# imdea-software/legosnark

Measured on AMD Instinct MI355X. Metric: alt_bn128 G1 MSM point-scalar pairs/s at n=2^20, higher is better.
Workload: dtype u32 limbs (254-bit Montgomery integers)

## Files before the change

### legosnark_amd/csrc/msm.hip

```cpp
#include <hip/hip_runtime.h>
#include <stdint.h>
#include <stdio.h>
#include <stdlib.h>
#include <string.h>
#include <algorithm>
#include <type_traits>
#include <vector>

#include "curves.h"
#include "fp29x2l.h"
#include "fs29.h"
#include "glv.h"
#include "msm.h"
#include "msm_plan.h"

namespace lsa {


template <class F, int K>
__global__ __launch_bounds__(256) void k_normalize(const Jac<F> *__restrict__ in, Aff<F> *__restrict__ out, size_t n) {
    size_t t = (size_t)blockIdx.x * blockDim.x + threadIdx.x;
    size_t base = t * K;
    if (base >= n) return;
    F prod[K];
// ... 397 lines not shown
    const size_t lo = (size_t)t * tile;
    for (uint32_t il = threadIdx.x; il < tile; il += 1024) {
        const size_t i = lo + il;
        if (i >= n) break;
        const uint32_t seg = segment_of(segs, (uint32_t)i);
        const uint32_t local = (uint32_t)i - segs.off[seg];
        wide_digits(scalars[i], pl, seg * B, [&](unsigned k, int32_t sd) {
            if (sd != 0) {
                const uint32_t b = (uint32_t)(sd < 0 ? -sd : sd) - 1;
                const uint32_t ent = (local + k * win_stride) | (sd < 0 ? 0x80000000u : 0u);
                if (REC == 1) ((uint64_t *)out)[atomicAdd(&base[b >> 7], 1u)] = ((uint64_t)(b & 127u) << 32) | ent;
                else if (REC == 2) ((uint32_t *)out)[atomicAdd(&base[b >> 6], 1u)] = (ent & 0x81ffffffu) | ((b & 63u) << 25);
                else ((uint32_t *)out)[atomicAdd(&base[b], 1u)] = ent;
            }
        });
    }
}

__device__ __forceinline__ uint32_t lds_inc_rank(uint32_t *counters, uint32_t idx) {
    const uint32_t first = (uint32_t)__builtin_amdgcn_readfirstlane((int)idx);
    const uint64_t active = __ballot(1), same = __ballot(idx == first);
    if (same == active) {
        const uint32_t rank = __builtin_amdgcn_mbcnt_hi((uint32_t)(active >> 32), __builtin_amdgcn_mbcnt_lo((uint32_t)active, 0u));
        uint32_t base = 0;
        if (rank == 0) base = atomicAdd(&counters[first], (uint32_t)__popcll(active));
        return (uint32_t)__builtin_amdgcn_readfirstlane((int)base) + rank;
    }
    return atomicAdd(&counters[idx], 1u);
}
__global__ __launch_bounds__(1024) void k_partition(const Fr *__restrict__ scalars, size_t n, SegList segs, WidePlan pl, uint32_t B, uint32_t Bc,
                                                    CoarseMap cm, uint32_t pitch, const uint16_t *__restrict__ tile_hist,
                                                    const uint32_t *__restrict__ hist_c, uint32_t *__restrict__ offs_c,
                                                    const uint32_t *__restrict__ tile_base, uint32_t *__restrict__ recs) {
    __builtin_amdgcn_s_setprio(3);
    extern __shared__ __attribute__((aligned(16))) uint32_t stage[];
    __shared__ uint32_t lstart[PART_SEGS + 1], lcur[PART_SEGS], gdst[PART_SEGS], wtot[2][PART_SEGS / 64];
    const uint32_t t = xcd_tile(blockIdx.x, gridDim.x);
    const unsigned lane = threadIdx.x & 63, wv = threadIdx.x >> 6;
    {
        uint32_t gv = 0, lv = 0;
        if (threadIdx.x < Bc) { gv = hist_c[threadIdx.x]; lv = tile_hist[(size_t)t * pitch + threadIdx.x]; }
        uint32_t gi = gv, li = lv;
#pragma unroll
        for (int d = 1; d < 64; d <<= 1) {
            const uint32_t a = __shfl_up(gi, d, 64), b = __shfl_up(li, d, 64);
            if ((int)lane >= d) { gi += a; li += b; }
        }
        if (wv < PART_SEGS / 64 && lane == 63) { wtot[0][wv] = gi; wtot[1][wv] = li; }
        __syncthreads();
        if (threadIdx.x < Bc) {
            uint32_t gex = gi - gv, lex = li - lv;
            for (unsigned w = 0; w < wv; w++) { gex += wtot[0][w]; lex += wtot[1][w]; }
            lstart[threadIdx.x] = lex;
            lcur[threadIdx.x] = lex;
            gdst[threadIdx.x] = gex + tile_base[(size_t)t * pitch + threadIdx.x];
            if (blockIdx.x == 0) offs_c[threadIdx.x] = gex;
            if (threadIdx.x == Bc - 1) lstart[Bc] = lex + lv;
        }
    }
    __syncthreads();
    const size_t lo = (size_t)t * PART_TILE;
    const uint32_t fine_bits = cm.sh_hi;
    const uint32_t tlow = t & ((1u << (16 - fine_bits)) - 1);
    for (uint32_t j = 0; j < PART_TILE / 1024; j++) {
        const uint32_t il = threadIdx.x + j * 1024;
        const size_t i = lo + il;
        if (i >= n) break;
        const uint32_t seg = segment_of(segs, (uint32_t)i);
        wide_digits(scalars[i], pl, seg * B, [&](unsigned k, int32_t sd) {
            if (sd != 0) {
                const uint32_t b = (uint32_t)(sd < 0 ? -sd : sd) - 1;
                const uint32_t pos = atomicAdd(&lcur[cm.bin(b)], 1u);
                stage[pos] = (tlow << (16 + fine_bits)) | (cm.fine(b) << 16) | (k << 12) | (sd < 0 ? 0x800u : 0u) | il;
            }
        });
    }
    __syncthreads();
    for (uint32_t sg = threadIdx.x >> 5; sg < Bc; sg += 32) {
        const uint32_t a = lstart[sg], e = lstart[sg + 1], g = gdst[sg];
        for (uint32_t x = a + (lane & 31); x < e; x += 32) recs[g + (x - a)] = stage[x];
    }
}

__global__ __launch_bounds__(1024) void k_fine_sort_part(const uint32_t *__restrict__ recs, const uint32_t *__restrict__ offs_c,
                                                         const uint32_t *__restrict__ hist_c, const uint32_t *__restrict__ tile_base,
                                                         uint32_t pitch, uint32_t T, CoarseMap cm, SegList segs, uint32_t win_stride, uint32_t stage_cap,
                                                         uint32_t *__restrict__ entries, uint32_t *__restrict__ hist, uint32_t *__restrict__ offs) {
    __builtin_amdgcn_s_setprio(3);
    extern __shared__ __attribute__((aligned(16))) uint32_t sm[];
    __shared__ uint32_t wsum[16];
    const uint32_t sg = blockIdx.x, lo = offs_c[sg], ns = hist_c[sg];
    const uint32_t fine_bits = cm.sh_hi, FM = 1u << fine_bits, fmask = FM - 1, tbits = 16 - fine_bits;
    const uint32_t F = 1u << cm.bits(sg), bucket0 = cm.first(sg);
    uint32_t *cnt = sm, *cur = sm + FM, *col = sm + 2 * FM, *stage = col + T + 1;
    const unsigned lane = threadIdx.x & 63, wv = threadIdx.x >> 6;
    for (uint32_t x = threadIdx.x; x < F; x += 1024) cnt[x] = 0;
    for (uint32_t x = threadIdx.x; x < T; x += 1024) col[x] = tile_base[(size_t)x * pitch + sg];
    if (threadIdx.x == 0) col[T] = ns;
    auto scan_counters = [&]() {
        const uint32_t per = (F + 1023) >> 10, f0 = threadIdx.x * per;
        uint32_t sum = 0;
        for (uint32_t q = 0; q < per; q++) if (f0 + q < F) sum += cnt[f0 + q];
        uint32_t incl = sum;
#pragma unroll
        for (int d = 1; d < 64; d <<= 1) {
            const uint32_t u = __shfl_up(incl, d, 64);
            if ((int)lane >= d) incl += u;
        }
        if (lane == 63) wsum[wv] = incl;
        __syncthreads();
        uint32_t run = incl - sum;
        for (unsigned w = 0; w < wv; w++) run += wsum[w];
        for (uint32_t q = 0; q < per; q++) {
            if (f0 + q >= F) break;
            const uint32_t c = cnt[f0 + q];
            cur[f0 + q] = run;
            hist[(size_t)bucket0 + f0 + q] = c;
            offs[(size_t)bucket0 + f0 + q] = lo + run;
            run += c;
        }
    };
    auto entry_of = [&](uint32_t r, uint32_t p2) {
        uint32_t a = 0, e = (T + (1u << tbits) - 1) >> tbits;
        while (e - a > 1) {
            const uint32_t m = (a + e) >> 1;
            if (col[m << tbits] <= p2) a = m; else e = m;
        }
        const uint32_t i = ((a << tbits) | (r >> (16 + fine_bits))) * PART_TILE + (r & 0x7ffu);
        const uint32_t local = i - segs.off[segment_of(segs, i)];
        return (local + ((r >> 12) & 15u) * win_stride) | ((r & 0x800u) << 20);
    };
    if (ns <= stage_cap) {
        constexpr uint32_t NR = PART_STAGE / 1024;
        uint32_t r[NR];
#pragma unroll
        for (uint32_t u = 0; u < NR; u++) { const uint32_t p2 = threadIdx.x + u * 1024; r[u] = p2 < ns ? recs[lo + p2] : 0u; }
        __syncthreads();
        uint16_t rk[NR];
#pragma unroll
        for (uint32_t u = 0; u < NR; u++) {
            rk[u] = 0;
            if (threadIdx.x + u * 1024 < ns) rk[u] = (uint16_t)atomicAdd(&cnt[(r[u] >> 16) & fmask], 1u);
        }
        __syncthreads();
        scan_counters();
        __syncthreads();
#pragma unroll
        for (uint32_t u = 0; u < NR; u++) {
            const uint32_t p2 = threadIdx.x + u * 1024;
            if (p2 < ns) stage[cur[(r[u] >> 16) & fmask] + rk[u]] = entry_of(r[u], p2);
        }
        __syncthreads();
        for (uint32_t x = threadIdx.x; x < ns; x += 1024) entries[lo + x] = stage[x];
        return;
    }
    __syncthreads();
    constexpr uint32_t UNR = 8;
    for (uint32_t p0 = threadIdx.x; p0 < ns; p0 += 1024 * UNR) {
        uint32_t r[UNR];
#pragma unroll
        for (uint32_t u = 0; u < UNR; u++) { const uint32_t p2 = p0 + u * 1024; r[u] = p2 < ns ? recs[lo + p2] : 0u; }
#pragma unroll
        for (uint32_t u = 0; u < UNR; u++) if (p0 + u * 1024 < ns) (void)lds_inc_rank(cnt, (r[u] >> 16) & fmask);
    }
    __syncthreads();
    scan_counters();
    __syncthreads();
    for (uint32_t p0 = threadIdx.x; p0 < ns; p0 += 1024 * UNR) {
        uint32_t r[UNR];
#pragma unroll
        for (uint32_t u = 0; u < UNR; u++) { const uint32_t p2 = p0 + u * 1024; r[u] = p2 < ns ? recs[lo + p2] : 0u; }
#pragma unroll
        for (uint32_t u = 0; u < UNR; u++) {
            const uint32_t p2 = p0 + u * 1024;
            if (p2 >= ns) break;
            entries[lo + lds_inc_rank(cur, (r[u] >> 16) & fmask)] = entry_of(r[u], p2);
        }
    }
}

template <class Rec>
struct RecOps;
template <>
struct RecOps<uint64_t> {
    static constexpr uint32_t NF = 128;
    static __device__ __forceinline__ uint32_t fine(uint64_t r) { return (uint32_t)(r >> 32); }
    static __device__ __forceinline__ uint32_t entry(uint64_t r) { return (uint32_t)r; }
};
template <>
struct RecOps<uint32_t> {
    static constexpr uint32_t NF = 64;
    static __device__ __forceinline__ uint32_t fine(uint32_t r) { return (r >> 25) & 63u; }
    static __device__ __forceinline__ uint32_t entry(uint32_t r) { return r & 0x81ffffffu; }
};
template <class Rec>
__global__ __launch_bounds__(1024) void k_fine_sort(const Rec *__restrict__ recs, const uint32_t *__restrict__ offs_c,
                                                    const uint32_t *__restrict__ hist_c, uint32_t *__restrict__ entries,
                                                    uint32_t *__restrict__ hist, uint32_t *__restrict__ offs) {
    using O = RecOps<Rec>;
    constexpr uint32_t NF = O::NF;
    __shared__ uint32_t cnt[NF], cur[NF];
    const uint32_t bin = blockIdx.x, lo = offs_c[bin], n = hist_c[bin];
    if (threadIdx.x < NF) cnt[threadIdx.x] = 0;
    __syncthreads();
    for (uint32_t j = threadIdx.x; j < n; j += 1024) atomicAdd(&cnt[O::fine(recs[lo + j])], 1u);
    __syncthreads();
    if (threadIdx.x < 64) {
        constexpr uint32_t PER = NF / 64;
        uint32_t c[PER], tot = 0;
#pragma unroll
        for (uint32_t q = 0; q < PER; q++) { c[q] = cnt[PER * threadIdx.x + q]; tot += c[q]; }
        uint32_t incl = tot;
#pragma unroll
        for (int d = 1; d < 64; d <<= 1) {
            uint32_t t = __shfl_up(incl, d, 64);
            if ((int)threadIdx.x >= d) incl += t;
        }
        uint32_t ex = incl - tot;
#pragma unroll
        for (uint32_t q = 0; q < PER; q++) {
            cur[PER * threadIdx.x + q] = ex;
            hist[(size_t)bin * NF + PER * threadIdx.x + q] = c[q];
            offs[(size_t)bin * NF + PER * threadIdx.x + q] = lo + ex;
            ex += c[q];
        }
    }
    __syncthreads();
    for (uint32_t j = threadIdx.x; j < n; j += 1024) {
        const Rec r = recs[lo + j];
        const uint32_t pos = atomicAdd(&cur[O::fine(r)], 1u);
        entries[lo + pos] = O::entry(r);
    }
}

__device__ __forceinline__ uint32_t size_bin(uint32_t cnt, uint32_t bin_shift) { return ((cnt - 1) >> bin_shift) + 1; }
template <class C>
__global__ __launch_bounds__(256) void k_size_hist(const uint32_t *__restrict__ hist, uint32_t nb, uint32_t thr, uint32_t *__restrict__ bin_count,
                                                   uint32_t group_size, uint32_t bin_shift) {
    bin_count += (group_size ? (blockIdx.x * 2048u) / group_size : 0u) * SIZE_BINS;
    __shared__ uint32_t lcnt[SIZE_BINS];
    for (uint32_t t = threadIdx.x; t < SIZE_BINS; t += 256) lcnt[t] = 0;
    __syncthreads();
    const uint32_t base = blockIdx.x * 2048 + threadIdx.x;
#pragma unroll
    for (int j = 0; j < 8; j++) {
        uint32_t g = base + j * 256;
        if (g < nb) { uint32_t cnt = hist[g]; if (cnt > 0 && cnt <= thr) atomicAdd(&lcnt[size_bin(cnt, bin_shift)], 1u); }
    }
    __syncthreads();
    for (uint32_t t = threadIdx.x; t < SIZE_BINS; t += 256) if (lcnt[t]) atomicAdd(&bin_count[t], lcnt[t]);
}
__global__ __launch_bounds__(256) void k_size_scan(const uint32_t *__restrict__ bin_count, uint32_t *__restrict__ bin_start, uint32_t ngroups) {
    __shared__ uint32_t lds[4];
    uint32_t carry = 0;
    for (uint32_t gidx = 0; gidx < ngroups; gidx++) {
        const uint32_t *bc = bin_count + gidx * SIZE_BINS;
        uint32_t *bs = bin_start + gidx * SIZE_BINS;
        uint32_t v[4], s = 0;
#pragma unroll
        for (int j = 0; j < 4; j++) {
            int bin = (int)SIZE_BINS - 1 - (int)(threadIdx.x * 4 + j);
            v[j] = (bin >= 1) ? bc[bin] : 0;
            s += v[j];
        }
        uint32_t tot;
        uint32_t run = carry + block_exclusive_scan_256(s, lds, &tot);
#pragma unroll
        for (int j = 0; j < 4; j++) {
            int bin = (int)SIZE_BINS - 1 - (int)(threadIdx.x * 4 + j);
            if (bin >= 1) bs[bin] = run;
            run += v[j];
        }
        carry += tot;
    }
    if (threadIdx.x == 0) bin_start[0] = carry;
}
template <class C>
__global__ __launch_bounds__(256) void k_size_scatter(const uint32_t *__restrict__ hist, uint32_t nb, uint32_t thr, const uint32_t *__restrict__ bin_start,
                                                      uint32_t *__restrict__ bin_cursor, uint32_t *__restrict__ perm,
                                                      uint32_t *__restrict__ heavy_list, uint32_t *__restrict__ heavy_count,
                                                      typename C::Acc *__restrict__ buckets, uint32_t group_size, uint32_t bin_shift,
                                                      uint32_t split) {
    const uint32_t goff = (group_size ? (blockIdx.x * 2048u) / group_size : 0u) * SIZE_BINS;
    bin_start += goff;
    bin_cursor += goff;
    __shared__ uint32_t lcnt[SIZE_BINS];
    for (uint32_t t = threadIdx.x; t < SIZE_BINS; t += 256) lcnt[t] = 0;
    __syncthreads();
    const uint32_t base = blockIdx.x * 2048 + threadIdx.x;
    uint32_t cnt[8], rank[8];
#pragma unroll
    for (int j = 0; j < 8; j++) {
        uint32_t g = base + j * 256;
        cnt[j] = 0; rank[j] = 0;
        if (g < nb) {
            cnt[j] = hist[g];
            if (cnt[j] == 0) { for (uint32_t h = 0; h < split; h++) buckets[(size_t)g * split + h] = C::inf(); }
            else if (cnt[j] > thr) heavy_list[atomicAdd(heavy_count, 1u)] = g;
            else rank[j] = atomicAdd(&lcnt[size_bin(cnt[j], bin_shift)], 1u);
        }
    }
    __syncthreads();
    for (uint32_t t = threadIdx.x; t < SIZE_BINS; t += 256) {
        uint32_t c = lcnt[t];
        lcnt[t] = c ? atomicAdd(&bin_cursor[t], c) : 0;
    }
    __syncthreads();
#pragma unroll
    for (int j = 0; j < 8; j++) {
        uint32_t g = base + j * 256;
        if (g < nb && cnt[j] > 0 && cnt[j] <= thr) {
            const uint32_t bin = size_bin(cnt[j], bin_shift);
            perm[bin_start[bin] + lcnt[bin] + rank[j]] = g;
        }
    }
}

typedef uint32_t u32x4 __attribute__((ext_vector_type(4)));
template <class B> struct RawBase {
    static_assert(sizeof(B) % 16 == 0, "packed bases are whole 16-byte vectors");
    u32x4 q[sizeof(B) / 16];
};
template <class B>
__device__ __forceinline__ RawBase<B> load_base16(const B *__restrict__ p) {
    const u32x4 *src = reinterpret_cast<const u32x4 *>(p);
    RawBase<B> r;
#pragma unroll
    for (int i = 0; i < (int)(sizeof(B) / 16); i++) r.q[i] = src[i];
    return r;
}
template <class B>
__device__ __forceinline__ B packed_base(RawBase<B> r) {
    B b;
    uint32_t *dst = reinterpret_cast<uint32_t *>(&b);
#pragma unroll
    for (int i = 0; i < (int)(sizeof(B) / 16); i++) {
        asm("" : "+v"(r.q[i]));
        dst[4 * i] = r.q[i].x; dst[4 * i + 1] = r.q[i].y; dst[4 * i + 2] = r.q[i].z; dst[4 * i + 3] = r.q[i].w;
    }
    return b;
}
template <class C> struct RotatedLoads { static constexpr bool value = true; };
template <> struct RotatedLoads<CurveG2> { static constexpr bool value = false; };
template <class C, uint32_t ACC_SPLIT, bool ROTATED = RotatedLoads<C>::value>
__device__ __forceinline__ void accumulate_body(const typename C::Base *__restrict__ bases, const uint32_t *__restrict__ entries,
                                                const uint32_t *__restrict__ offs, const uint32_t *__restrict__ hist,
                                                const uint32_t *__restrict__ perm, const uint32_t *__restrict__ nperm,
                                                typename C::Acc *__restrict__ buckets) {
    uint32_t t = blockIdx.x * blockDim.x + threadIdx.x;
    if (t >= *nperm * ACC_SPLIT) return;
    const uint32_t g = perm[t / ACC_SPLIT], part = t % ACC_SPLIT;
    const uint32_t cnt = hist[g];
    const uint32_t *e = entries + offs[g];
    constexpr bool ENDO = ACC_SPLIT != 1;
    typename C::Acc acc = C::inf();
    if constexpr (!ROTATED) {
        if (part < cnt) {
            uint32_t v = e[part];
            typename C::Base cur = bases[v & 0x3fffffffu];
            static_assert(!C::HEAD || ROTATED, "the affine + affine head is written for the rotated loop only");
            for (uint32_t j = part; j < cnt; j += ACC_SPLIT) {
                uint32_t vn = v;
                typename C::Base nxt = cur;
                if (j + ACC_SPLIT < cnt) { vn = e[j + ACC_SPLIT]; nxt = bases[vn & 0x3fffffffu]; }
                acc = C::template madd<ENDO>(acc, cur, (v >> 31) != 0, ((v >> 30) & 1) != 0);
                v = vn;
                cur = nxt;
            }
        }
    } else if (part < cnt) {
        const uint32_t last = part + (cnt - 1 - part) / ACC_SPLIT * ACC_SPLIT;
        auto word = [&](uint32_t k) { return e[k < last ? k : last]; };
        auto base = [&](uint32_t w) { return load_base16(bases + (w & 0x3fffffffu)); };
        uint32_t j = part;
        uint32_t v = word(j), vn = word(j + ACC_SPLIT);
        RawBase<typename C::Base> cur;
        if constexpr (C::HEAD) {
            const uint32_t v2 = word(j + 2 * ACC_SPLIT), v3 = word(j + 3 * ACC_SPLIT);
            const RawBase<typename C::Base> r0 = base(v), r1 = base(vn), r2 = base(v2);
            const typename C::Base b0 = packed_base(r0), b1 = packed_base(r1);
            cur = r0;
            if (j + ACC_SPLIT < cnt && C::head_ok(b0, b1)) {
                acc = C::template madd_head<ENDO>(b0, (v >> 31) != 0, ((v >> 30) & 1) != 0, b1, (vn >> 31) != 0, ((vn >> 30) & 1) != 0);
                j += 2 * ACC_SPLIT;
                v = v2;
                vn = v3;
                cur = r2;
            }
        } else {
            cur = base(v);
        }
        for (; j < cnt; j += ACC_SPLIT) {
            const uint32_t vnn = word(j + 2 * ACC_SPLIT);
            const RawBase<typename C::Base> nxt = base(vn);
            acc = C::template madd<ENDO>(acc, packed_base(cur), (v >> 31) != 0, ((v >> 30) & 1) != 0);
            v = vn;
            vn = vnn;
            cur = nxt;
        }
    }
    buckets[(size_t)g * ACC_SPLIT + part] = acc;
}
template <class C, uint32_t ACC_SPLIT>
__global__ __launch_bounds__(256) void k_accumulate(const typename C::Base *__restrict__ bases, const uint32_t *__restrict__ entries,
                                                    const uint32_t *__restrict__ offs, const uint32_t *__restrict__ hist,
                                                    const uint32_t *__restrict__ perm, const uint32_t *__restrict__ nperm,
                                                    typename C::Acc *__restrict__ buckets) {
    accumulate_body<C, ACC_SPLIT>(bases, entries, offs, hist, perm, nperm, buckets);
}
__global__ __launch_bounds__(256) __attribute__((amdgpu_waves_per_eu(2, 2))) void k_accumulate_g2_occ2(
    const CurveG2::Base *__restrict__ bases, const uint32_t *__restrict__ entries, const uint32_t *__restrict__ offs,
    const uint32_t *__restrict__ hist, const uint32_t *__restrict__ perm, const uint32_t *__restrict__ nperm, CurveG2::Acc *__restrict__ buckets) {
    accumulate_body<CurveG2, 1u>(bases, entries, offs, hist, perm, nperm, buckets);
}

__global__ __launch_bounds__(256) void k_accumulate_g2_pair(const AffPackedG2 *__restrict__ bases, const uint32_t *__restrict__ entries,
                                                            const uint32_t *__restrict__ offs, const uint32_t *__restrict__ hist,
                                                            const uint32_t *__restrict__ perm, const uint32_t *__restrict__ nperm,
                                                            XYZZ29x2 *__restrict__ buckets) {
    const uint32_t t = blockIdx.x * blockDim.x + threadIdx.x, pr = t >> 1, part = t & 1;
    if (pr >= *nperm) return;
    const uint32_t g = perm[pr];
    const uint32_t cnt = hist[g];
    const uint32_t *e = entries + offs[g];
    struct Half { uint32_t x[8], y[8]; };
    auto fetch = [&](uint32_t v) {
        const AffPackedG2 &b = bases[v & 0x3fffffffu];
        Half h;
#pragma unroll
        for (int i = 0; i < 8; i++) { h.x[i] = b.w[part][i]; h.y[i] = b.w[2 + part][i]; }
        return h;
    };
    XyzzE<F29h> acc = XyzzE<F29h>::inf();
    uint32_t v = e[0];
    Half cur = fetch(v);
    for (uint32_t j = 0; j < cnt; j++) {
        uint32_t vn = v;
        Half nxt = cur;
        if (j + 1 < cnt) { vn = e[j + 1]; nxt = fetch(vn); }
        AffE<F29h> q = {{F29::unpack256(cur.x)}, {F29::unpack256(cur.y)}};
        if (!q.is_inf()) {
            if (v >> 31) q.y = sub_k<1>(F29h::zero(), q.y);
            acc = g2_madd(acc, q);
        }
        v = vn;
        cur = nxt;
    }
    F29 *o = reinterpret_cast<F29 *>(&buckets[g]);
    o[part] = acc.X.v;
    o[2 + part] = acc.Y.v;
    o[4 + part] = acc.ZZ.v;
    o[6 + part] = acc.ZZZ.v;
}

template <class A>
__device__ __forceinline__ A shfl_down_acc(const A &p, unsigned delta) {
    A r;
    constexpr int NW = sizeof(A) / 4;
    const uint32_t *src = reinterpret_cast<const uint32_t *>(&p);
    uint32_t *dst = reinterpret_cast<uint32_t *>(&r);
#pragma unroll
    for (int i = 0; i < NW; i++) dst[i] = __shfl_down(src[i], delta, 64);
    return r;
}

enum TailKernel { TAIL_HEAVY, TAIL_REDUCE1_LANE, TAIL_REDUCE2_LANE };
template <class C, TailKernel K> struct PairedAdd { static constexpr bool value = false; };
template <> struct PairedAdd<CurveG1, TAIL_HEAVY> { static constexpr bool value = true; };
template <> struct PairedAdd<CurveG1, TAIL_REDUCE1_LANE> { static constexpr bool value = true; };

template <class C, bool PAIRED = false>
__device__ __forceinline__ typename C::Acc wave_sum(typename C::Acc v, unsigned lane) {
    for (unsigned d = 32; d >= 1; d >>= 1) {
        typename C::Acc t = shfl_down_acc(v, d);
        if (lane + d < 64) v = C::template add<PAIRED>(v, t);
    }
    return v;
}

__global__ __launch_bounds__(256) void k_heavy_plan(const uint32_t *__restrict__ hist, const uint32_t *__restrict__ heavy_list,
                                                    const uint32_t *__restrict__ heavy_count, uint32_t *__restrict__ chunk_off) {
    __shared__ uint32_t lds[4];
    __shared__ uint32_t s_chunk;
    const uint32_t nh = *heavy_count;
    uint32_t carry = 0;
    for (uint32_t base = 0; base < nh; base += 256) {
        uint32_t h = base + threadIdx.x;
        uint32_t tot;
        (void)block_exclusive_scan_256(h < nh ? hist[heavy_list[h]] : 0, lds, &tot);
        carry += tot;
    }
    if (threadIdx.x == 0) {
        uint32_t chunk = HEAVY_CHUNK;
        while (chunk < 4096u && carry / (2 * chunk) >= 2048u) chunk *= 2;
        s_chunk = chunk;
    }
    __syncthreads();
    const uint32_t chunk = s_chunk;
    carry = 0;
    for (uint32_t base = 0; base < nh; base += 256) {
        uint32_t h = base + threadIdx.x;
        uint32_t v = h < nh ? (hist[heavy_list[h]] + chunk - 1) / chunk : 0;
        uint32_t tot;
        uint32_t ex = block_exclusive_scan_256(v, lds, &tot);
        if (h < nh) chunk_off[h] = carry + ex;
        carry += tot;
    }
    if (threadIdx.x == 0) { chunk_off[nh] = carry; chunk_off[nh + 1] = chunk; }
}

template <class C>
__global__ __launch_bounds__(64) void k_accumulate_heavy(const typename C::Base *__restrict__ bases, const uint32_t *__restrict__ entries,
                                                         const uint32_t *__restrict__ offs, const uint32_t *__restrict__ hist,
                                                         const uint32_t *__restrict__ heavy_list, const uint32_t *__restrict__ heavy_count,
                                                         const uint32_t *__restrict__ chunk_off, typename C::Acc *__restrict__ partials) {
    const uint32_t nh = *heavy_count;
    if (nh == 0) return;
    const uint32_t total = chunk_off[nh], chunk = chunk_off[nh + 1];
    const unsigned lane = threadIdx.x;
    for (uint32_t v = blockIdx.x; v < total; v += gridDim.x) {
        uint32_t lo = 0, hi = nh;
        while (hi - lo > 1) { uint32_t mid = (lo + hi) >> 1; if (chunk_off[mid] <= v) lo = mid; else hi = mid; }
        const uint32_t g = heavy_list[lo];
        const uint32_t cnt = hist[g];
        const uint32_t start = (v - chunk_off[lo]) * chunk;
        const uint32_t end = start + chunk < cnt ? start + chunk : cnt;
        const uint32_t *e = entries + offs[g];
        typename C::Acc acc = C::inf();
        uint32_t j = start + lane;
        if constexpr (!RotatedLoads<C>::value) {
            for (; j < end; j += 64) {
                uint32_t w = e[j];
                acc = C::madd(acc, bases[w & 0x3fffffffu], (w >> 31) != 0, ((w >> 30) & 1) != 0);
            }
        } else if (j < end) {
            const uint32_t last = j + (end - 1 - j) / 64 * 64;
            auto word = [&](uint32_t k) { return e[k < last ? k : last]; };
            uint32_t w = word(j), wn = word(j + 64);
            RawBase<typename C::Base> cur = load_base16(bases + (w & 0x3fffffffu));
            for (; j < end; j += 64) {
                const uint32_t wnn = word(j + 128);
                const RawBase<typename C::Base> nxt = load_base16(bases + (wn & 0x3fffffffu));
                acc = C::madd(acc, packed_base(cur), (w >> 31) != 0, ((w >> 30) & 1) != 0);
                w = wn;
                wn = wnn;
                cur = nxt;
            }
        }
        acc = wave_sum<C, PairedAdd<C, TAIL_HEAVY>::value>(acc, lane);
        if (lane == 0) partials[v] = acc;
    }
}

template <class C>
__global__ __launch_bounds__(64) void k_heavy_finish(const uint32_t *__restrict__ heavy_list, const uint32_t *__restrict__ heavy_count,
                                                     const uint32_t *__restrict__ chunk_off, const typename C::Acc *__restrict__ partials,
                                                     typename C::Acc *__restrict__ buckets, uint32_t split) {
    const uint32_t nh = *heavy_count;
    unsigned lane = threadIdx.x;
    for (uint32_t h = blockIdx.x; h < nh; h += gridDim.x) {
        typename C::Acc acc = C::inf();
        for (uint32_t v = chunk_off[h] + lane; v < chunk_off[h + 1]; v += 64) acc = C::add(acc, partials[v]);
        acc = wave_sum<C>(acc, lane);
        if (lane == 0) {
            buckets[(size_t)heavy_list[h] * split] = acc;
            for (uint32_t x = 1; x < split; x++) buckets[(size_t)heavy_list[h] * split + x] = C::inf();
        }
    }
}

template <class A>
__device__ __forceinline__ A select_acc(uint32_t mask, const A &a, const A &b) {
    A r;
    const uint32_t *pa = reinterpret_cast<const uint32_t *>(&a), *pb = reinterpret_cast<const uint32_t *>(&b);
    uint32_t *pr = reinterpret_cast<uint32_t *>(&r);
#pragma unroll
    for (int i = 0; i < (int)(sizeof(A) / 4); i++) pr[i] = (pa[i] & mask) | (pb[i] & ~mask);
    return r;
}
template <class A>
__device__ __forceinline__ void quadwave_weighted(A &acc, A &run, unsigned log_mult, unsigned lane) {
    const unsigned q = lane & 3, qi = lane >> 2;
    A s = A::inf();
#pragma unroll 1
    for (unsigned step = 0; step < 9; step++) {
        if (step == 4) {
            s = (qi == 0) ? A::inf() : run;
#pragma unroll 1
            for (unsigned i = 0; i < log_mult; i++) s = quad_dbl(s, q);
        }
        uint32_t m_run = step < 4 ? 0xffffffffu : 0u, m_s = step == 4 ? 0xffffffffu : 0u;
// ... 570 lines not shown
    (void)hipFree(tmp);
    if (rc) return rc;
    if (e != hipSuccess) { set_error("precompute_windows: %s", hipGetErrorString(e)); return LSA_ERR_HIP; }
    return LSA_OK;
}
template <class F>
int precompute_window_step(void *d_table, size_t n, void *d_tmp, unsigned k, hipStream_t st) {
    using C = typename CurveOf<F>::type;
    const TableGrid grid = table_grid(n);
    if (n == 0 || k == 0 || k >= grid.ncopies) return LSA_OK;
    typename C::Base *tbl = (typename C::Base *)d_table;
    hipLaunchKernelGGL((k_shift_window<C>), dim3((unsigned)((n + 255) / 256)), dim3(256), 0, st, tbl + (size_t)(k - 1) * n, (Jac<F> *)d_tmp, n, grid.pos[k] - grid.pos[k - 1]);
    return prepare_bases<F>((const Jac<F> *)d_tmp, tbl + (size_t)k * n, n, st);
}
template int precompute_window_step<Fq>(void *, size_t, void *, unsigned, hipStream_t);
template int precompute_window_step<Fq2>(void *, size_t, void *, unsigned, hipStream_t);
template int precompute_windows<Fq>(void *, size_t, hipStream_t);
template int precompute_windows<Fq2>(void *, size_t, hipStream_t);

unsigned msm_field_mults_per_pair(size_t n, size_t table_n) {
    if (table_n && n >= switches().table_use_min) return wide_plan(table_n, n, 1, switches()).nwin * 10;
    return 16 * 10 + 8;
}

template <class A>
struct MsmBuffers {
    uint32_t *hist, *heavy_count, *offs, *bsum, *bin_count, *bin_start, *bin_cursor, *perm;
    int32_t *digits;
    uint16_t *rank, *tile_hist;
    uint32_t *tile_base, *entries, *heavy_list, *chunk_off;
    A *hpart;
    void *recs;
    uint32_t *hist_c, *offs_c;
    A *buckets, *wave_out, *window_sums;
    void *res;

    MsmBuffers(const PipelinePlan &p, void *front_ws, void *tail_ws) {
        char *ws = (char *)front_ws, *tws = (char *)tail_ws;
        hist = (uint32_t *)(ws + p.front[F_HIST]);
        heavy_count = hist + p.nb;
        offs = (uint32_t *)(ws + p.front[F_OFFS]);
        bsum = (uint32_t *)(ws + p.front[F_BSUM]);
        bin_count = (uint32_t *)(ws + p.front[F_BINS]);
        bin_start = bin_count + SIZE_BINS;
        bin_cursor = bin_start + SIZE_BINS;
        perm = (uint32_t *)(ws + p.front[F_PERM]);
        digits = (int32_t *)(ws + p.front[F_DIGITS]);
        rank = (uint16_t *)(ws + p.front[F_RANK]);
        tile_hist = (uint16_t *)(ws + p.front[F_THIST]);
        tile_base = (uint32_t *)(ws + p.front[F_TBASE]);
        entries = (uint32_t *)(ws + p.front[F_ENTRIES]);
        heavy_list = (uint32_t *)(ws + p.front[F_HEAVY]);
        chunk_off = (uint32_t *)(ws + p.front[F_CHOFF]);
        hpart = (A *)(ws + p.front[F_HPART]);
        recs = ws + p.front[F_RECS];
        hist_c = p.fine ? (uint32_t *)(ws + p.front[F_CHIST]) : hist;
        offs_c = p.fine ? (uint32_t *)(ws + p.front[F_COFFS]) : offs;
        buckets = (A *)(tws + p.tail[T_BUCKETS]);
        wave_out = (A *)(tws + p.tail[T_WAVE]);
        window_sums = (A *)(tws + p.tail[T_WIN]);
        res = tws + p.tail[T_RES];
    }
};

struct Marks {
    hipEvent_t *ev;
    void operator()(int i, hipStream_t s) const { if (ev) (void)hipEventRecord(ev[i], s); }
};

template <class C>
static void launch_sort(const PipelinePlan &p, const MsmBuffers<typename C::Acc> &b, const Fr *d_scalars, const SegList &segs, hipStream_t st,
                        const Marks &mark) {
    const size_t n = p.n;
    if (p.wide) {
        hipLaunchKernelGGL(k_hist_wide, dim3(p.wtiles), dim3(1024), p.lds_hist_wide, st, d_scalars, n, segs, p.pl, p.B, p.Bc, p.cm, p.pitch, p.wtile, b.tile_hist);
        mark(1, st);
        hipLaunchKernelGGL(k_tile_scan_rows, dim3((p.Bc + 31) / 32), dim3(1024), 0, st, b.tile_hist, p.Bc, p.wtiles, p.pitch, b.tile_base, b.hist_c, b.heavy_count,
                           b.bin_count, (uint32_t)(3 * SIZE_BINS));
        mark(2, st);
        if (p.part) {
            hipLaunchKernelGGL(k_partition, dim3(p.wtiles), dim3(1024), p.lds_partition, st, d_scalars, n, segs, p.pl, p.B, p.Bc, p.cm, p.pitch,
                               b.tile_hist, b.hist_c, b.offs_c, b.tile_base, (uint32_t *)b.recs);
            hipLaunchKernelGGL(k_fine_sort_part, dim3(p.Bc), dim3(1024), p.lds_fine_sort_part, st, (const uint32_t *)b.recs, b.offs_c, b.hist_c,
                               b.tile_base, p.pitch, p.wtiles, p.cm, segs, p.win_stride, p.stage_cap, b.entries, b.hist, b.offs);
        } else if (p.rec32) {
            hipLaunchKernelGGL(k_scatter_wide<2>, dim3(p.wtiles), dim3(1024), p.lds_scatter_wide, st, d_scalars, n, segs, p.pl, p.B, p.Bc, p.pitch, p.wtile, b.hist_c, b.offs_c, b.tile_base, b.recs, p.win_stride);
            hipLaunchKernelGGL(k_fine_sort<uint32_t>, dim3(p.Bc), dim3(1024), 0, st, (const uint32_t *)b.recs, b.offs_c, b.hist_c, b.entries, b.hist, b.offs);
        } else if (p.fine) {
            hipLaunchKernelGGL(k_scatter_wide<1>, dim3(p.wtiles), dim3(1024), p.lds_scatter_wide, st, d_scalars, n, segs, p.pl, p.B, p.Bc, p.pitch, p.wtile, b.hist_c, b.offs_c, b.tile_base, b.recs, p.win_stride);
            hipLaunchKernelGGL(k_fine_sort<uint64_t>, dim3(p.Bc), dim3(1024), 0, st, (const uint64_t *)b.recs, b.offs_c, b.hist_c, b.entries, b.hist, b.offs);
        } else {
            hipLaunchKernelGGL(k_scatter_wide<0>, dim3(p.wtiles), dim3(1024), p.lds_scatter_wide, st, d_scalars, n, segs, p.pl, p.B, p.Bc, p.pitch, p.wtile, b.hist_c, b.offs_c, b.tile_base, (void *)b.entries, p.win_stride);
        }
        mark(3, st);
    } else {
        hipLaunchKernelGGL((k_digits<C::GLV>), dim3((unsigned)((n + 255) / 256)), dim3(256), 0, st, d_scalars, n, p.c, p.nwin, b.digits);
        hipLaunchKernelGGL(k_rank, dim3(p.ntiles, p.nwin), dim3(1024), p.lds_rank, st, b.digits, p.nv, p.B, p.ntiles, b.rank, b.tile_hist, 0u);
        hipLaunchKernelGGL(k_tile_scan, dim3((p.nb + 255) / 256), dim3(256), 0, st, b.tile_hist, p.B, p.ntiles, p.nb, b.tile_base, b.hist);
        mark(1, st);
        hipLaunchKernelGGL(k_scan_sums, dim3(p.scan_blocks), dim3(256), 0, st, b.hist, p.nb, b.bsum);
        hipLaunchKernelGGL(k_scan_blocks, dim3(1), dim3(256), 0, st, b.bsum, p.scan_blocks);
        hipLaunchKernelGGL(k_scan_final, dim3(p.scan_blocks), dim3(256), 0, st, b.hist, b.bsum, p.nb, b.offs);
        mark(2, st);
        hipLaunchKernelGGL(k_scatter, dim3(p.ntiles, p.nwin), dim3(1024), p.lds_scatter, st, b.digits, b.rank, b.offs, b.tile_base, p.nv, n, p.B, p.ntiles, b.entries, 0u);
        mark(3, st);
    }
}

template <class C>
static int launch_accumulate(const PipelinePlan &p, const MsmBuffers<typename C::Acc> &b, const typename C::Base *d_bases, hipStream_t st, const Marks &mark) {
    constexpr bool g2 = std::is_same<C, CurveG2>::value;
    if (!p.wide || p.reuse_sort) {
        HIPCHK(hipMemsetAsync(b.heavy_count, 0, 4, st));
        HIPCHK(hipMemsetAsync(b.bin_count, 0, (size_t)3 * SIZE_BINS * 4, st));
    }
    const unsigned sb = (p.nb + 2047) / 2048;
    const uint32_t gsz = 0u, ngroups = 1;
    hipLaunchKernelGGL((k_size_hist<C>), dim3(sb), dim3(256), 0, st, b.hist, p.nb, p.heavy_threshold, b.bin_count, gsz, p.bin_shift);
    hipLaunchKernelGGL(k_size_scan, dim3(1), dim3(256), 0, st, b.bin_count, b.bin_start, ngroups);
    hipLaunchKernelGGL((k_size_scatter<C>), dim3(sb), dim3(256), 0, st, b.hist, p.nb, p.heavy_threshold, b.bin_start, b.bin_cursor, b.perm, b.heavy_list, b.heavy_count, b.buckets, gsz, p.bin_shift, p.split);
    mark(4, st);
    const dim3 one_lane((p.nb + 255) / 256), two_lanes((p.nb * 2 + 255) / 256);
    if (g2 && p.g2_pair) {
        if constexpr (g2) hipLaunchKernelGGL(k_accumulate_g2_pair, two_lanes, dim3(256), 0, st, d_bases, b.entries, b.offs, b.hist, b.perm, b.bin_start, b.buckets);
    } else if (g2 && p.split == 1) {
        if constexpr (g2) hipLaunchKernelGGL(k_accumulate_g2_occ2, one_lane, dim3(256), 0, st, d_bases, b.entries, b.offs, b.hist, b.perm, b.bin_start, b.buckets);
    } else if (p.split == 1) {
        hipLaunchKernelGGL((k_accumulate<C, 1u>), one_lane, dim3(256), 0, st, d_bases, b.entries, b.offs, b.hist, b.perm, b.bin_start, b.buckets);
    } else {
        hipLaunchKernelGGL((k_accumulate<C, 2u>), two_lanes, dim3(256), 0, st, d_bases, b.entries, b.offs, b.hist, b.perm, b.bin_start, b.buckets);
    }
    hipLaunchKernelGGL(k_heavy_plan, dim3(1), dim3(256), 0, st, b.hist, b.heavy_list, b.heavy_count, b.chunk_off);
    hipLaunchKernelGGL((k_accumulate_heavy<C>), dim3(4096), dim3(64), 0, st, d_bases, b.entries, b.offs, b.hist,
                       b.heavy_list, b.heavy_count, b.chunk_off, b.hpart);
    hipLaunchKernelGGL((k_heavy_finish<C>), dim3(256), dim3(64), 0, st, b.heavy_list, b.heavy_count, b.chunk_off, b.hpart, b.buckets, p.split);
    mark(5, st);
    return LSA_OK;
}

template <class C>
static int launch_tail(const PipelinePlan &p, const MsmBuffers<typename C::Acc> &b, Jac<typename C::Field> *d_out, hipStream_t tail, bool inline_tail,
                       bool lane_l1, TailBuf &tb, TailBuf &prev, const Marks &mark) {
    using A = typename C::Acc;
    using J = Jac<typename C::Field>;
    constexpr bool g1 = std::is_same<C, CurveG1>::value;
    if (p.big)
        hipLaunchKernelGGL((k_reduce1_lane<C>), dim3(p.kw * ((p.T + 63) / 64)), dim3(64), 0, tail, b.buckets, p.B, p.L, p.split, b.wave_out);
    else
        hipLaunchKernelGGL((k_reduce1<C>), dim3(p.kw * p.wpw), dim3(64), 0, tail, b.buckets, p.B, p.L, p.logL, p.wpw, p.split, b.wave_out);
    A *lvl_in = b.wave_out, *lvl_out = b.window_sums;
    uint32_t m = p.wpw, lm = p.big ? p.logL : p.logL + 4;
    J *res = inline_tail ? d_out : (J *)b.res;
    const auto level = [&](bool lane) {
        const uint32_t m_out = (m + 15) / 16;
        if (lane) hipLaunchKernelGGL((k_reduce2_lane<C>), dim3((m_out + 63) / 64), dim3(64), 0, tail, lvl_in, m, m_out, lm, lvl_out);
        else hipLaunchKernelGGL((k_reduce2<C>), dim3(p.kw * m_out), dim3(64), 0, tail, lvl_in, m, m_out, lm, lvl_out);
        std::swap(lvl_in, lvl_out);
        m = m_out;
        lm += 4;
    };
    level(lane_l1);
    if (p.bits_tail) {
        uint32_t nbits = 0;
        while ((1u << nbits) < m) nbits++;
        const uint32_t G = (m + 511) / 512;
        A *part = lvl_out;
        A *weighted = part + (size_t)(nbits + 1) * G;
        hipLaunchKernelGGL((k_reduce_bits_a<C>), dim3(nbits + 1, G), dim3(512), 0, tail, lvl_in, m, nbits, G, part);
        hipLaunchKernelGGL((k_reduce_bits_b<C>), dim3(nbits + 1), dim3(64), 0, tail, part, nbits, G, lm, weighted);
        mark(6, tail);
        hipLaunchKernelGGL((k_reduce_bits_c<C>), dim3(1), dim3(64), 0, tail, weighted, nbits + 1, res);
    } else {
        while (m > 1) level(false);
        mark(6, tail);
        if (p.wide && p.nseg > 1) {
            if constexpr (g1) hipLaunchKernelGGL(k_emit_g1, dim3(p.nseg), dim3(64), 0, tail, lvl_in, res);
            else hipLaunchKernelGGL(k_emit_g2, dim3(p.nseg), dim3(64), 0, tail, lvl_in, res);
        } else if constexpr (g1) {
            hipLaunchKernelGGL(k_fold_quad, dim3(1), dim3(64), 0, tail, lvl_in, p.kw, p.c, res);
        } else {
            hipLaunchKernelGGL(k_fold_quad_g2, dim3(1), dim3(64), 0, tail, lvl_in, p.kw, p.c, res);
        }
    }
    if (!inline_tail) {
        int rc = publish_order_large(tb, prev, tail);
        if (rc) return rc;
        hipLaunchKernelGGL(k_publish, dim3(1), dim3(256), 0, tail, (const uint32_t *)res, (uint32_t *)d_out, (unsigned)(p.nseg * sizeof(J) / 4));
    }
    mark(7, tail);
    return LSA_OK;
}

static int plan_error(const PipelinePlan &p) {
    switch (p.status) {
    case PLAN_OK: return LSA_OK;
    case PLAN_N_TOO_LARGE: set_error("msm: n too large (%zu)", p.n); break;
    case PLAN_SEGMENTS_NEED_COPIES: set_error("msm: segmented calls need bases with pre-shifted copies"); break;
    case PLAN_TABLE_TOO_LARGE: set_error("msm: base table too large for 30-bit entries"); break;
    case PLAN_BIN_SPACE: set_error("msm: %u segments of %u buckets exceed the bin space", p.nseg, p.B); break;
    }
    return LSA_ERR_INVALID;
}

template <class F>
static int msm_pipeline(const void *d_bases_v, size_t first, const Fr *d_scalars, const SegList &segs, Jac<F> *d_out, hipStream_t st,
                        size_t table_stride, bool reuse_sort = false, bool blocking = false) {
    using C = typename CurveOf<F>::type;
    using A = typename C::Acc;
    const typename C::Base *d_bases = (const typename C::Base *)d_bases_v + first;
    const MsmShape shape = {std::is_same<C, CurveG1>::value ? 1 : 2, sizeof(A), sizeof(Jac<F>), C::GLV, segs.off[segs.nseg], segs.nseg,
                            table_stride, blocking, reuse_sort};
    const PipelinePlan p = plan_pipeline(shape, switches());
    int rc = plan_error(p);
    if (rc) return rc;
    if (g_ws.ensure(p.front.total) != 0) { set_error("msm: workspace allocation of %zu bytes failed", p.front.total); return LSA_ERR_NOMEM; }
// ... 101 lines not shown
```

### legosnark_amd/csrc/msm_plan.h

```cpp
#pragma once
#include <stdint.h>
#include <stddef.h>
#include "bn254_constants.h"
#include "fp.h"

namespace lsa {

struct WidePlan {
    unsigned nwin;
    unsigned c;
    unsigned copy_step;
    unsigned start[32];
    unsigned width[32];
};

struct TableGrid {
    unsigned ncopies;
    unsigned pos[33];
};
inline TableGrid table_grid(size_t n_table) {
    TableGrid t;
    const unsigned nbig = n_table >= ((size_t)6 << 20) ? 12u : 13u;
    const unsigned base = 255 / nbig, rem = 255 % nbig;
    unsigned bit = 0;
    for (unsigned k = 0; k < nbig; k++) {
        const unsigned w = base + (k < rem ? 1u : 0u);
        t.pos[2 * k] = bit;
        t.pos[2 * k + 1] = bit + (w + 1) / 2;
        bit += w;
    }
    t.ncopies = 2 * nbig;
    t.pos[t.ncopies] = 255;
    return t;
}

inline WidePlan wide_plan_for(size_t n_table, bool big) {
    const TableGrid t = table_grid(n_table);
    WidePlan pl = {};
    pl.copy_step = big ? 2 : 1;
    pl.nwin = t.ncopies / pl.copy_step;
    pl.c = 0;
    for (unsigned k = 0; k < pl.nwin; k++) {
        pl.start[k] = t.pos[k * pl.copy_step];
        pl.width[k] = t.pos[(k + 1) * pl.copy_step] - pl.start[k];
        if (pl.width[k] > pl.c) pl.c = pl.width[k];
    }
    return pl;
}

#define SORT_TILE 32768u
#define SCAN_PER_BLOCK 2048
#define WIDE_FINE_BITS 7u
#define MSM_MAX_SEGMENTS 64u
#define PART_TILE 2048u
#define PART_SEGS 768u
#define PART_STAGE 28672u
#define SIZE_BINS 1025
#define HEAVY_CHUNK 512u

constexpr uint32_t LDS_MAX_BIN_WORDS = 131072;
constexpr uint32_t LDS_MAX_BIN_HALVES = 65536;
constexpr uint32_t LDS_MAX_PARTITION = 13 * PART_TILE * 4;
constexpr uint32_t LDS_MAX_FINE_SORT_PART = 155648;

struct SegList {
    uint32_t nseg;
    uint32_t off[MSM_MAX_SEGMENTS + 1];
};

struct CoarseMap {
    uint32_t half, sh_lo, sh_hi, nlo;
    LSA_HD uint32_t bin(uint32_t b) const { return b < half ? b >> sh_lo : nlo + ((b - half) >> sh_hi); }
    LSA_HD uint32_t fine(uint32_t b) const { return b < half ? b & ((1u << sh_lo) - 1) : (b - half) & ((1u << sh_hi) - 1); }
    LSA_HD uint32_t first(uint32_t bin_) const { return bin_ < nlo ? bin_ << sh_lo : half + ((bin_ - nlo) << sh_hi); }
    LSA_HD uint32_t bits(uint32_t bin_) const { return bin_ < nlo ? sh_lo : sh_hi; }
};

inline unsigned msm_window_bits(size_t n) {
    unsigned lg = 0;
    while ((size_t(1) << (lg + 1)) <= n) lg++;
    int c = (int)lg - 4;
    if (c < 8) c = 8;
    if (c > 16) c = 16;
    return (unsigned)c;
}

inline unsigned num_windows(unsigned c) { return (255 + c - 1) / c; }

inline uint32_t wide_tile(uint32_t nwin, size_t n) {
    if (n <= 4096) return 256u;
    if (n <= 16384) return 1024u;
    return nwin > 15 ? 2048u : 4096u;
}

struct MsmSwitches {
    bool no_rec32 = false;
    bool no_part = false;
    uint32_t wide_split = 1;
    bool g2_pair = false;
    bool no_reduce_bits = false;
    bool no_lane_l1 = false;
    bool g2_lane_l1 = false;
    size_t wide_big_min = (size_t)1 << 16;
    size_t table_use_min = 1;
};

struct MsmShape {
    int group;
    size_t acc_bytes;
    size_t jac_bytes;
    bool glv;
    size_t n;
    uint32_t nseg;
    size_t table_stride;
    bool blocking, reuse_sort;
};

enum PlanStatus {
    PLAN_OK = 0,
    PLAN_N_TOO_LARGE,
    PLAN_SEGMENTS_NEED_COPIES,
    PLAN_TABLE_TOO_LARGE,
    PLAN_BIN_SPACE,
};

inline size_t align_up(size_t x, size_t a) { return (x + a - 1) / a * a; }

struct WsRegion { size_t off, bytes; };
enum FrontRegion {
    F_HIST,
    F_OFFS,
    F_BSUM,
    F_BINS,
    F_PERM,
    F_DIGITS,
    F_RANK,
    F_THIST,
    F_TBASE,
    F_ENTRIES,
    F_HEAVY,
    F_CHOFF,
    F_HPART,
    F_RECS,
    F_CHIST,
    F_COFFS,
    F_REGIONS
// ... 219 lines not shown
```

Measured before the change: 852.7 million.

## Fuse bucket size histogram into fine sort and heavy plan into accumulate

Computes the bucket size-bin histogram inside k_fine_sort_part from the LDS counters and folds the bin-start scan into k_size_scatter, removing the k_size_hist and k_size_scan launches and one pass over hist. The heavy-bucket planning runs as an extra workgroup of k_accumulate instead of a separate single-block launch. This cuts launch count and serial tiny kernels, but it adds global atomics into bin_count and assumes bin_count is zeroed beforehand and that 1024 threads match the bin count.

```diff
diff --git a/legosnark_amd/csrc/msm.hip b/legosnark_amd/csrc/msm.hip
--- a/legosnark_amd/csrc/msm.hip
+++ b/legosnark_amd/csrc/msm.hip
@@ -503,10 +503,13 @@
     }
 }
 
+__device__ __forceinline__ uint32_t size_bin(uint32_t cnt, uint32_t bin_shift) { return ((cnt - 1) >> bin_shift) + 1; }
+
 __global__ __launch_bounds__(1024) void k_fine_sort_part(const uint32_t *__restrict__ recs, const uint32_t *__restrict__ offs_c,
                                                          const uint32_t *__restrict__ hist_c, const uint32_t *__restrict__ tile_base,
                                                          uint32_t pitch, uint32_t T, CoarseMap cm, SegList segs, uint32_t win_stride, uint32_t stage_cap,
-                                                         uint32_t *__restrict__ entries, uint32_t *__restrict__ hist, uint32_t *__restrict__ offs) {
+                                                         uint32_t *__restrict__ entries, uint32_t *__restrict__ hist, uint32_t *__restrict__ offs,
+                                                         uint32_t thr, uint32_t bin_shift, uint32_t *__restrict__ bin_count) {
     __builtin_amdgcn_s_setprio(3);
     extern __shared__ __attribute__((aligned(16))) uint32_t sm[];
     __shared__ uint32_t wsum[16];
@@ -551,6 +554,19 @@
         const uint32_t local = i - segs.off[segment_of(segs, i)];
         return (local + ((r >> 12) & 15u) * win_stride) | ((r & 0x800u) << 20);
     };
+    static_assert(SIZE_BINS - 1 == 1024, "one bin per thread of k_fine_sort_part, and FM >= 2^10 counters to hold them");
+    auto bin_sizes = [&]() {
+        __syncthreads();
+        cur[threadIdx.x] = 0;
+        __syncthreads();
+        for (uint32_t x = threadIdx.x; x < F; x += 1024) {
+            const uint32_t c = cnt[x];
+            if (c > 0 && c <= thr) atomicAdd(&cur[size_bin(c, bin_shift) - 1], 1u);
+        }
+        __syncthreads();
+        const uint32_t c = cur[threadIdx.x];
+        if (c) atomicAdd(&bin_count[threadIdx.x + 1], c);
+    };
     if (ns <= stage_cap) {
         constexpr uint32_t NR = PART_STAGE / 1024;
         uint32_t r[NR];
@@ -573,6 +589,7 @@
         }
         __syncthreads();
         for (uint32_t x = threadIdx.x; x < ns; x += 1024) entries[lo + x] = stage[x];
+        bin_sizes();
         return;
     }
     __syncthreads();
@@ -598,6 +615,7 @@
             entries[lo + lds_inc_rank(cur, (r[u] >> 16) & fmask)] = entry_of(r[u], p2);
         }
     }
+    bin_sizes();
 }
 
 template <class Rec>
@@ -654,7 +672,6 @@
     }
 }
 
-__device__ __forceinline__ uint32_t size_bin(uint32_t cnt, uint32_t bin_shift) { return ((cnt - 1) >> bin_shift) + 1; }
 template <class C>
 __global__ __launch_bounds__(256) void k_size_hist(const uint32_t *__restrict__ hist, uint32_t nb, uint32_t thr, uint32_t *__restrict__ bin_count,
                                                    uint32_t group_size, uint32_t bin_shift) {
@@ -696,8 +713,9 @@
     }
     if (threadIdx.x == 0) bin_start[0] = carry;
 }
-template <class C>
-__global__ __launch_bounds__(256) void k_size_scatter(const uint32_t *__restrict__ hist, uint32_t nb, uint32_t thr, const uint32_t *__restrict__ bin_start,
+template <class C, bool SCAN = false>
+__global__ __launch_bounds__(256) void k_size_scatter(const uint32_t *__restrict__ hist, uint32_t nb, uint32_t thr, const uint32_t *__restrict__ bin_count,
+                                                      uint32_t *__restrict__ bin_start,
                                                       uint32_t *__restrict__ bin_cursor, uint32_t *__restrict__ perm,
                                                       uint32_t *__restrict__ heavy_list, uint32_t *__restrict__ heavy_count,
                                                       typename C::Acc *__restrict__ buckets, uint32_t group_size, uint32_t bin_shift,
@@ -706,16 +724,44 @@
     bin_start += goff;
     bin_cursor += goff;
     __shared__ uint32_t lcnt[SIZE_BINS];
-    for (uint32_t t = threadIdx.x; t < SIZE_BINS; t += 256) lcnt[t] = 0;
-    __syncthreads();
+    __shared__ uint32_t lstart[SCAN ? SIZE_BINS : 1];
     const uint32_t base = blockIdx.x * 2048 + threadIdx.x;
     uint32_t cnt[8], rank[8];
+    if constexpr (SCAN) {
+#pragma unroll
+        for (int j = 0; j < 8; j++) { const uint32_t g = base + j * 256; cnt[j] = g < nb ? hist[g] : 0u; }
+    }
+    for (uint32_t t = threadIdx.x; t < SIZE_BINS; t += 256) lcnt[t] = 0;
+    if constexpr (SCAN) {
+        __shared__ uint32_t lds[4];
+        uint32_t v[4], s = 0;
+#pragma unroll
+        for (int j = 0; j < 4; j++) {
+            const int bin = (int)SIZE_BINS - 1 - (int)(threadIdx.x * 4 + j);
+            v[j] = (bin >= 1) ? bin_count[bin] : 0;
+            s += v[j];
+        }
+        uint32_t tot;
+        uint32_t run = block_exclusive_scan_256(s, lds, &tot);
+#pragma unroll
+        for (int j = 0; j < 4; j++) {
+            const int bin = (int)SIZE_BINS - 1 - (int)(threadIdx.x * 4 + j);
+            if (bin >= 1) {
+                lstart[bin] = run;
+                if (blockIdx.x == 0) bin_start[bin] = run;
+            }
+            run += v[j];
+        }
+        if (blockIdx.x == 0 && threadIdx.x == 0) bin_start[0] = tot;
+    }
+    __syncthreads();
 #pragma unroll
     for (int j = 0; j < 8; j++) {
         uint32_t g = base + j * 256;
-        cnt[j] = 0; rank[j] = 0;
+        if constexpr (!SCAN) cnt[j] = 0;
+        rank[j] = 0;
         if (g < nb) {
-            cnt[j] = hist[g];
+            if constexpr (!SCAN) cnt[j] = hist[g];
             if (cnt[j] == 0) { for (uint32_t h = 0; h < split; h++) buckets[(size_t)g * split + h] = C::inf(); }
             else if (cnt[j] > thr) heavy_list[atomicAdd(heavy_count, 1u)] = g;
             else rank[j] = atomicAdd(&lcnt[size_bin(cnt[j], bin_shift)], 1u);
@@ -732,7 +778,7 @@
         uint32_t g = base + j * 256;
         if (g < nb && cnt[j] > 0 && cnt[j] <= thr) {
             const uint32_t bin = size_bin(cnt[j], bin_shift);
-            perm[bin_start[bin] + lcnt[bin] + rank[j]] = g;
+            perm[(SCAN ? lstart[bin] : bin_start[bin]) + lcnt[bin] + rank[j]] = g;
         }
     }
 }
@@ -822,11 +868,17 @@
     }
     buckets[(size_t)g * ACC_SPLIT + part] = acc;
 }
-template <class C, uint32_t ACC_SPLIT>
+__device__ __forceinline__ void heavy_plan_body(const uint32_t *__restrict__ hist, const uint32_t *__restrict__ heavy_list,
+                                                const uint32_t *__restrict__ heavy_count, uint32_t *__restrict__ chunk_off);
+template <class C, uint32_t ACC_SPLIT, bool PLAN = false>
 __global__ __launch_bounds__(256) void k_accumulate(const typename C::Base *__restrict__ bases, const uint32_t *__restrict__ entries,
                                                     const uint32_t *__restrict__ offs, const uint32_t *__restrict__ hist,
                                                     const uint32_t *__restrict__ perm, const uint32_t *__restrict__ nperm,
-                                                    typename C::Acc *__restrict__ buckets) {
+                                                    typename C::Acc *__restrict__ buckets, const uint32_t *__restrict__ heavy_list,
+                                                    const uint32_t *__restrict__ heavy_count, uint32_t *__restrict__ chunk_off) {
+    if constexpr (PLAN) {
+        if (blockIdx.x == gridDim.x - 1) { heavy_plan_body(hist, heavy_list, heavy_count, chunk_off); return; }
+    }
     accumulate_body<C, ACC_SPLIT>(bases, entries, offs, hist, perm, nperm, buckets);
 }
 __global__ __launch_bounds__(256) __attribute__((amdgpu_waves_per_eu(2, 2))) void k_accumulate_g2_occ2(
@@ -899,8 +951,8 @@
     return v;
 }
 
-__global__ __launch_bounds__(256) void k_heavy_plan(const uint32_t *__restrict__ hist, const uint32_t *__restrict__ heavy_list,
-                                                    const uint32_t *__restrict__ heavy_count, uint32_t *__restrict__ chunk_off) {
+__device__ __forceinline__ void heavy_plan_body(const uint32_t *__restrict__ hist, const uint32_t *__restrict__ heavy_list,
+                                                const uint32_t *__restrict__ heavy_count, uint32_t *__restrict__ chunk_off) {
     __shared__ uint32_t lds[4];
     __shared__ uint32_t s_chunk;
     const uint32_t nh = *heavy_count;
@@ -911,23 +963,23 @@
         (void)block_exclusive_scan_256(h < nh ? hist[heavy_list[h]] : 0, lds, &tot);
         carry += tot;
     }
-    if (threadIdx.x == 0) {
-        uint32_t chunk = HEAVY_CHUNK;
-        while (chunk < 4096u && carry / (2 * chunk) >= 2048u) chunk *= 2;
-        s_chunk = chunk;
-    }
+    if (threadIdx.x == 0) s_chunk = heavy_chunk_size(carry);
     __syncthreads();
     const uint32_t chunk = s_chunk;
     carry = 0;
     for (uint32_t base = 0; base < nh; base += 256) {
         uint32_t h = base + threadIdx.x;
-        uint32_t v = h < nh ? (hist[heavy_list[h]] + chunk - 1) / chunk : 0;
+        uint32_t v = h < nh ? heavy_chunks_of(hist[heavy_list[h]], chunk) : 0;
         uint32_t tot;
         uint32_t ex = block_exclusive_scan_256(v, lds, &tot);
         if (h < nh) chunk_off[h] = carry + ex;
         carry += tot;
     }
     if (threadIdx.x == 0) { chunk_off[nh] = carry; chunk_off[nh + 1] = chunk; }
+}
+__global__ __launch_bounds__(256) void k_heavy_plan(const uint32_t *__restrict__ hist, const uint32_t *__restrict__ heavy_list,
+                                                    const uint32_t *__restrict__ heavy_count, uint32_t *__restrict__ chunk_off) {
+    heavy_plan_body(hist, heavy_list, heavy_count, chunk_off);
 }
 
 template <class C>
@@ -1664,7 +1716,8 @@
             hipLaunchKernelGGL(k_partition, dim3(p.wtiles), dim3(1024), p.lds_partition, st, d_scalars, n, segs, p.pl, p.B, p.Bc, p.cm, p.pitch,
                                b.tile_hist, b.hist_c, b.offs_c, b.tile_base, (uint32_t *)b.recs);
             hipLaunchKernelGGL(k_fine_sort_part, dim3(p.Bc), dim3(1024), p.lds_fine_sort_part, st, (const uint32_t *)b.recs, b.offs_c, b.hist_c,
-                               b.tile_base, p.pitch, p.wtiles, p.cm, segs, p.win_stride, p.stage_cap, b.entries, b.hist, b.offs);
+                               b.tile_base, p.pitch, p.wtiles, p.cm, segs, p.win_stride, p.stage_cap, b.entries, b.hist, b.offs,
+                               p.heavy_threshold, p.bin_shift, b.bin_count);
         } else if (p.rec32) {
             hipLaunchKernelGGL(k_scatter_wide<2>, dim3(p.wtiles), dim3(1024), p.lds_scatter_wide, st, d_scalars, n, segs, p.pl, p.B, p.Bc, p.pitch, p.wtile, b.hist_c, b.offs_c, b.tile_base, b.recs, p.win_stride);
             hipLaunchKernelGGL(k_fine_sort<uint32_t>, dim3(p.Bc), dim3(1024), 0, st, (const uint32_t *)b.recs, b.offs_c, b.hist_c, b.entries, b.hist, b.offs);
@@ -1698,21 +1751,32 @@
     }
     const unsigned sb = (p.nb + 2047) / 2048;
     const uint32_t gsz = 0u, ngroups = 1;
-    hipLaunchKernelGGL((k_size_hist<C>), dim3(sb), dim3(256), 0, st, b.hist, p.nb, p.heavy_threshold, b.bin_count, gsz, p.bin_shift);
-    hipLaunchKernelGGL(k_size_scan, dim3(1), dim3(256), 0, st, b.bin_count, b.bin_start, ngroups);
-    hipLaunchKernelGGL((k_size_scatter<C>), dim3(sb), dim3(256), 0, st, b.hist, p.nb, p.heavy_threshold, b.bin_start, b.bin_cursor, b.perm, b.heavy_list, b.heavy_count, b.buckets, gsz, p.bin_shift, p.split);
+    const bool fused = p.wide && p.part && !p.reuse_sort;
+    if (fused) {
+        hipLaunchKernelGGL((k_size_scatter<C, true>), dim3(sb), dim3(256), 0, st, b.hist, p.nb, p.heavy_threshold, b.bin_count, b.bin_start, b.bin_cursor, b.perm, b.heavy_list, b.heavy_count, b.buckets, gsz, p.bin_shift, p.split);
+    } else {
+        hipLaunchKernelGGL((k_size_hist<C>), dim3(sb), dim3(256), 0, st, b.hist, p.nb, p.heavy_threshold, b.bin_count, gsz, p.bin_shift);
+        hipLaunchKernelGGL(k_size_scan, dim3(1), dim3(256), 0, st, b.bin_count, b.bin_start, ngroups);
+        hipLaunchKernelGGL((k_size_scatter<C>), dim3(sb), dim3(256), 0, st, b.hist, p.nb, p.heavy_threshold, b.bin_count, b.bin_start, b.bin_cursor, b.perm, b.heavy_list, b.heavy_count, b.buckets, gsz, p.bin_shift, p.split);
+    }
     mark(4, st);
-    const dim3 one_lane((p.nb + 255) / 256), two_lanes((p.nb * 2 + 255) / 256);
+    const unsigned plan_wg = fused && !g2 ? 1u : 0u;
+    const dim3 one_lane((p.nb + 255) / 256 + plan_wg), two_lanes((p.nb * 2 + 255) / 256 + plan_wg);
+    const auto accumulate = [&](auto kernel, dim3 grid) {
+        hipLaunchKernelGGL(kernel, grid, dim3(256), 0, st, d_bases, b.entries, b.offs, b.hist, b.perm, b.bin_start, b.buckets, b.heavy_list, b.heavy_count, b.chunk_off);
+    };
     if (g2 && p.g2_pair) {
         if constexpr (g2) hipLaunchKernelGGL(k_accumulate_g2_pair, two_lanes, dim3(256), 0, st, d_bases, b.entries, b.offs, b.hist, b.perm, b.bin_start, b.buckets);
     } else if (g2 && p.split == 1) {
         if constexpr (g2) hipLaunchKernelGGL(k_accumulate_g2_occ2, one_lane, dim3(256), 0, st, d_bases, b.entries, b.offs, b.hist, b.perm, b.bin_start, b.buckets);
+    } else if (plan_wg) {
+        if constexpr (!g2) { if (p.split == 1) accumulate(k_accumulate<C, 1u, true>, one_lane); else accumulate(k_accumulate<C, 2u, true>, two_lanes); }
     } else if (p.split == 1) {
-        hipLaunchKernelGGL((k_accumulate<C, 1u>), one_lane, dim3(256), 0, st, d_bases, b.entries, b.offs, b.hist, b.perm, b.bin_start, b.buckets);
+        accumulate(k_accumulate<C, 1u>, one_lane);
     } else {
-        hipLaunchKernelGGL((k_accumulate<C, 2u>), two_lanes, dim3(256), 0, st, d_bases, b.entries, b.offs, b.hist, b.perm, b.bin_start, b.buckets);
-    }
-    hipLaunchKernelGGL(k_heavy_plan, dim3(1), dim3(256), 0, st, b.hist, b.heavy_list, b.heavy_count, b.chunk_off);
+        accumulate(k_accumulate<C, 2u>, two_lanes);
+    }
+    if (!plan_wg) hipLaunchKernelGGL(k_heavy_plan, dim3(1), dim3(256), 0, st, b.hist, b.heavy_list, b.heavy_count, b.chunk_off);
     hipLaunchKernelGGL((k_accumulate_heavy<C>), dim3(4096), dim3(64), 0, st, d_bases, b.entries, b.offs, b.hist,
                        b.heavy_list, b.heavy_count, b.chunk_off, b.hpart);
     hipLaunchKernelGGL((k_heavy_finish<C>), dim3(256), dim3(64), 0, st, b.heavy_list, b.heavy_count, b.chunk_off, b.hpart, b.buckets, p.split);
diff --git a/legosnark_amd/csrc/msm_plan.h b/legosnark_amd/csrc/msm_plan.h
--- a/legosnark_amd/csrc/msm_plan.h
+++ b/legosnark_amd/csrc/msm_plan.h
@@ -62,6 +62,13 @@
 constexpr uint32_t LDS_MAX_BIN_HALVES = 65536;
 constexpr uint32_t LDS_MAX_PARTITION = 13 * PART_TILE * 4;
 constexpr uint32_t LDS_MAX_FINE_SORT_PART = 155648;
+
+LSA_HD uint32_t heavy_chunk_size(uint32_t heavy_entries) {
+    uint32_t chunk = HEAVY_CHUNK;
+    while (chunk < 4096u && heavy_entries / (2 * chunk) >= 2048u) chunk *= 2;
+    return chunk;
+}
+LSA_HD uint32_t heavy_chunks_of(uint32_t cnt, uint32_t chunk) { return (cnt + chunk - 1) / chunk; }
 
 struct SegList {
     uint32_t nseg;
```

Result: faster. 861.3 million (median of 6 runs) (+1.0%).
